# dropbox/rust-brotli

Hardware: AMD Instinct MI355X
Metric: compress MB/s at q5 lgwin22 (higher is better)
Workload: dtype u8; 1 GPU; 64 MiB synthetic English-like text per GPU, quality=5, lgwin=22, one-shot BrotliEncoderCompress (H6), input and stream resident in HBM; input_bytes_total=67108864, compressed_bytes=16370400

## Files before the change

### rust-brotli_amd/csrc/metablock_device.h

```cpp
#ifndef BROTLI_MI355X_METABLOCK_DEVICE_H_
#define BROTLI_MI355X_METABLOCK_DEVICE_H_

#include "lz77_chain.h"
#include "metablock_types.h"

namespace brotli_mi355x {

struct BitSink {
  uint64_t* words;
  uint64_t pos;
  BR_DEV void put(uint32_t n_bits, uint64_t bits) {
    if (n_bits == 0) return;
    const uint32_t sh = (uint32_t)(pos & 63u);
    uint64_t* w = words + (pos >> 6);
    w[0] |= bits << sh;
    if (sh + n_bits > 64) w[1] |= bits >> (64 - sh);
    pos += n_bits;
  }
};

#if defined(BR_CODES_PROFILE) && !defined(BROTLI_HOST_EMU)
static __device__ unsigned long long g_codes_prof[32];
struct CodesPhaseClock {
  unsigned long long last;
// ... 467 lines not shown
        total_reps_non_zero += reps;
        count_reps_non_zero++;
      }
      i += reps;
    }
    use_rle_for_non_zero = total_reps_non_zero > count_reps_non_zero * 2;
    use_rle_for_zero = total_reps_zero > count_reps_zero * 2;
  }
  uint32_t n = *tree_size;
  for (uint32_t i = 0; i < new_length;) {
    const uint8_t value = depth[i];
    uint32_t reps = 1;
    if ((value != 0 && use_rle_for_non_zero) || (value == 0 && use_rle_for_zero)) {
      for (uint32_t k = i + 1; k < new_length && depth[k] == value; ++k) reps++;
    }
    uint32_t repetitions = reps;
    if (value == 0) {
      if (repetitions == 11) {
        tree[n] = 0;
        extra[n] = 0;
        n++;
        repetitions--;
      }
      if (repetitions < 3) {
        for (uint32_t r = 0; r < repetitions; ++r) {
          tree[n] = 0;
          extra[n] = 0;
          n++;
        }
      } else {
        const uint32_t start = n;
        repetitions -= 3;
        for (;;) {
          tree[n] = 17;
          extra[n] = (uint8_t)(repetitions & 0x7);
          n++;
          repetitions >>= 3;
          if (repetitions == 0) break;
          repetitions--;
        }
        br_reverse_u8(tree, start, n);
        br_reverse_u8(extra, start, n);
      }
    } else {
      if (previous_value != value) {
        tree[n] = value;
        extra[n] = 0;
        n++;
        repetitions--;
      }
      if (repetitions == 7) {
        tree[n] = value;
        extra[n] = 0;
        n++;
        repetitions--;
      }
      if (repetitions < 3) {
        for (uint32_t r = 0; r < repetitions; ++r) {
          tree[n] = value;
          extra[n] = 0;
          n++;
        }
      } else {
        const uint32_t start = n;
        repetitions -= 3;
        for (;;) {
          tree[n] = 16;
          extra[n] = (uint8_t)(repetitions & 0x3);
          n++;
          repetitions >>= 2;
          if (repetitions == 0) break;
          repetitions--;
        }
        br_reverse_u8(tree, start, n);
        br_reverse_u8(extra, start, n);
      }
      previous_value = value;
    }
    i += reps;
  }
  *tree_size = n;
}

BR_DEV uint16_t br_reverse_bits(uint32_t num_bits, uint16_t bits) {
#if !defined(BROTLI_HOST_EMU)
  if (num_bits != 0) return (uint16_t)(__builtin_bitreverse32((uint32_t)bits) >> (32u - num_bits));
#endif
  const uint32_t kLut[16] = {0x0, 0x8, 0x4, 0xc, 0x2, 0xa, 0x6, 0xe, 0x1, 0x9, 0x5, 0xd, 0x3, 0xb, 0x7, 0xf};
  uint32_t retval = kLut[bits & 0xf];
  for (uint32_t i = 4; i < num_bits; i += 4) {
    retval <<= 4;
    bits = (uint16_t)(bits >> 4);
    retval |= kLut[bits & 0xf];
  }
  retval >>= ((0u - num_bits) & 0x3u);
  return (uint16_t)retval;
}
BR_DEV void br_convert_bit_depths_to_symbols(const uint8_t* depth, uint32_t len, uint16_t* bits) {
  uint16_t bl_count[16];
  uint16_t next_code[16];
  for (int i = 0; i < 16; ++i) bl_count[i] = 0;
  for (uint32_t i = 0; i < len; ++i) bl_count[depth[i]]++;
  bl_count[0] = 0;
  next_code[0] = 0;
  int code = 0;
  for (int i = 1; i < 16; ++i) {
    code = (code + bl_count[i - 1]) << 1;
    next_code[i] = (uint16_t)code;
  }
  for (uint32_t i = 0; i < len; ++i)
    if (depth[i] != 0) bits[i] = br_reverse_bits(depth[i], next_code[depth[i]]++);
}
#if !defined(BROTLI_HOST_EMU)
BR_DEV void br_convert_bit_depths_to_symbols_coop(const uint8_t* depth, uint32_t len, uint16_t* bits) {
  const uint32_t lane = threadIdx.x & 63u;
  const unsigned long long below = (1ull << lane) - 1ull;
  uint32_t cnt = 0;
  for (uint32_t base = 0; base < len; base += 64) {
    const uint32_t i = base + lane;
    const uint32_t d = i < len ? depth[i] : 0u;
#pragma unroll
    for (uint32_t k = 1; k < 16; ++k) {
      const unsigned long long m = __ballot(d == k);
      if (lane == k) cnt += (uint32_t)__popcll(m);
    }
  }
  uint32_t code = 0, running = 0;
#pragma unroll
  for (uint32_t k = 1; k < 16; ++k) {
    const uint32_t c_prev = k == 1 ? 0u : (uint32_t)__shfl((int)cnt, (int)(k - 1), 64);
    code = (code + c_prev) << 1;
    if (lane == k) running = code;
  }
  for (uint32_t base = 0; base < len; base += 64) {
    const uint32_t i = base + lane;
    const uint32_t d = i < len ? depth[i] : 0u;
    const uint32_t next = (uint32_t)__shfl((int)running, (int)d, 64);
    uint32_t rank = 0;
#pragma unroll
    for (uint32_t k = 1; k < 16; ++k) {
      const unsigned long long m = __ballot(d == k);
      if (d == k) rank = (uint32_t)__popcll(m & below);
      if (lane == k) running += (uint32_t)__popcll(m);
    }
    if (d != 0) bits[i] = br_reverse_bits(d, (uint16_t)(next + rank));
  }
  __threadfence_block();
  __builtin_amdgcn_wave_barrier();
}
#endif

struct HuffmanScratch {
  HuffmanTree tree[2 * 704 + 2];
  uint8_t rle_tree[704];
  uint8_t rle_extra[704];
  uint8_t good_for_rle[704];
  uint8_t pad[8];
  HuffmanTree sort_tmp[704];
};

BR_DEV void br_store_huffman_tree(const uint8_t* depths, uint32_t num, HuffmanScratch* sc, BitSink& out) {
  const uint8_t kStorageOrder[18] = {1, 2, 3, 4, 0, 5, 17, 6, 16, 7, 8, 9, 10, 11, 12, 13, 14, 15};
  const uint8_t kSymbols[6] = {0, 7, 3, 2, 1, 15};
  const uint8_t kBitLengths[6] = {2, 4, 3, 2, 2, 4};
  uint32_t huffman_tree_size = 0;
  uint8_t code_length_bitdepth[18];
  uint16_t code_length_bitdepth_symbols[18];
  uint32_t huffman_tree_histogram[18];
  for (int i = 0; i < 18; ++i) {
    code_length_bitdepth[i] = 0;
    code_length_bitdepth_symbols[i] = 0;
    huffman_tree_histogram[i] = 0;
  }
  BR_PHASE_CLOCK();
  br_write_huffman_tree(depths, num, &huffman_tree_size, sc->rle_tree, sc->rle_extra);
  BR_PHASE(4);
  for (uint32_t i = 0; i < huffman_tree_size; ++i) huffman_tree_histogram[sc->rle_tree[i]]++;
  BR_PHASE(5);
  int num_codes = 0;
  uint32_t code = 0;
  for (uint32_t i = 0; i < 18; ++i) {
    if (huffman_tree_histogram[i] != 0) {
      if (num_codes == 0) {
        code = i;
        num_codes = 1;
      } else if (num_codes == 1) {
        num_codes = 2;
        break;
      }
    }
  }
  br_create_huffman_tree(huffman_tree_histogram, 18, 5, sc->tree, code_length_bitdepth);
  br_convert_bit_depths_to_symbols(code_length_bitdepth, 18, code_length_bitdepth_symbols);
  {
    uint32_t skip_some = 0;
    uint32_t codes_to_store = 18;
    if (num_codes > 1) {
      for (; codes_to_store > 0; --codes_to_store)
        if (code_length_bitdepth[kStorageOrder[codes_to_store - 1]] != 0) break;
    }
    if (code_length_bitdepth[kStorageOrder[0]] == 0 && code_length_bitdepth[kStorageOrder[1]] == 0) {
      skip_some = 2;
      if (code_length_bitdepth[kStorageOrder[2]] == 0) skip_some = 3;
    }
    out.put(2, skip_some);
    for (uint32_t i = skip_some; i < codes_to_store; ++i) {
      const uint32_t l = code_length_bitdepth[kStorageOrder[i]];
      out.put(kBitLengths[l], kSymbols[l]);
    }
  }
  if (num_codes == 1) code_length_bitdepth[code] = 0;
  BR_PHASE(6);
  for (uint32_t i = 0; i < huffman_tree_size; ++i) {
    const uint32_t ix = sc->rle_tree[i];
    out.put(code_length_bitdepth[ix], code_length_bitdepth_symbols[ix]);
    if (ix == 16) {
      out.put(2, sc->rle_extra[i]);
    } else if (ix == 17) {
      out.put(3, sc->rle_extra[i]);
    }
  }
  BR_PHASE(7);
}

BR_DEV void br_build_and_store_huffman_tree(const uint32_t* histogram, uint32_t histogram_length, uint32_t alphabet_size,
                                            HuffmanScratch* sc, uint8_t* depth, uint16_t* bits, BitSink& out, bool coop = false) {
  uint32_t count = 0;
  uint32_t s4[4] = {0, 0, 0, 0};
  uint32_t max_bits = 0;
  for (uint32_t i = 0; i < histogram_length; ++i) {
    if (histogram[i] != 0) {
      if (count < 4) {
        s4[count] = i;
      } else if (count > 4) {
        break;
      }
      count++;
    }
  }
  for (uint32_t c = alphabet_size - 1; c != 0; c >>= 1) max_bits++;
  if (count <= 1) {
    out.put(4, 1);
    out.put(max_bits, s4[0]);
    depth[s4[0]] = 0;
    bits[s4[0]] = 0;
    return;
  }
  for (uint32_t i = 0; i < histogram_length; ++i) depth[i] = 0;
  BR_PHASE_CLOCK();
  br_create_huffman_tree(histogram, histogram_length, 15, sc->tree, depth, coop ? sc->sort_tmp : nullptr);
  BR_PHASE(14);
#if !defined(BROTLI_HOST_EMU)
  if (coop) br_convert_bit_depths_to_symbols_coop(depth, histogram_length, bits); else
#endif
  br_convert_bit_depths_to_symbols(depth, histogram_length, bits);
  BR_PHASE(8);
  if (count <= 4) {
    out.put(2, 1);
    out.put(2, count - 1);
    for (uint32_t i = 0; i < count; ++i) {
      for (uint32_t j = i + 1; j < count; ++j) {
        if (depth[s4[j]] < depth[s4[i]]) {
          const uint32_t t = s4[j];
          s4[j] = s4[i];
          s4[i] = t;
        }
      }
    }
    for (uint32_t i = 0; i < count; ++i) out.put(max_bits, s4[i]);
    if (count == 4) out.put(1, depth[s4[0]] == 1 ? 1 : 0);
  } else {
    br_store_huffman_tree(depth, histogram_length, sc, out);
  }
}

BR_DEV uint32_t br_block_length_offset(uint32_t code) {
  const uint32_t kOffset[26] = {1,   5,   9,   13,  17,  25,  33,  41,  49,   65,   81,   97,   113,
                                145, 177, 209, 241, 305, 369, 497, 753, 1265, 2289, 4337, 8433, 16625};
  return kOffset[code];
}
BR_DEV uint32_t br_block_length_nbits(uint32_t code) {
  const uint8_t kNbits[26] = {2, 2, 2, 2, 3, 3, 3, 3, 4, 4, 4, 4, 5, 5, 5, 5, 6, 6, 7, 8, 9, 10, 11, 12, 13, 24};
  return kNbits[code];
}
BR_DEV uint32_t br_block_length_prefix_code(uint32_t len) {
  uint32_t code = len >= 177 ? (len >= 753 ? 20 : 14) : (len >= 41 ? 7 : 0);
  while (code < 25 && len >= br_block_length_offset(code + 1)) code++;
  return code;
}
struct BlockTypeCodeCalculator {
  uint32_t last_type, second_last_type;
};
BR_DEV uint32_t br_next_block_type_code(BlockTypeCodeCalculator& c, uint8_t type) {
  const uint32_t type_code = (type == c.last_type + 1) ? 1u : (type == c.second_last_type ? 0u : (uint32_t)type + 2u);
  c.second_last_type = c.last_type;
  c.last_type = type;
  return type_code;
}
BR_DEV void br_store_var_len_uint8(uint32_t n, BitSink& out) {
  if (n == 0) {
    out.put(1, 0);
  } else {
    const uint32_t nbits = br_log2_floor_nonzero(n);
    out.put(1, 1);
    out.put(3, nbits);
    out.put(nbits, n - (1u << nbits));
  }
}

struct BlockSplitCode {
  uint8_t type_depths[258];
  uint16_t type_bits[258];
  uint8_t length_depths[26];
  uint16_t length_bits[26];
};

BR_DEV uint64_t br_block_switch_bits(const BlockSplitCode& code, uint32_t typecode, uint32_t block_len, bool is_first_block,
                                     uint32_t* nbits_out) {
  uint64_t bits = 0;
  uint32_t n = 0;
  if (!is_first_block) {
    bits = code.type_bits[typecode];
    n = code.type_depths[typecode];
  }
  const uint32_t lencode = br_block_length_prefix_code(block_len);
  bits |= (uint64_t)code.length_bits[lencode] << n;
  n += code.length_depths[lencode];
  bits |= (uint64_t)(block_len - br_block_length_offset(lencode)) << n;
  n += br_block_length_nbits(lencode);
  *nbits_out = n;
  return bits;
}

BR_DEV uint32_t br_block_type_code_at(const uint8_t* types, uint32_t i) {
  const uint32_t type = types[i];
  const uint32_t last = i >= 1 ? types[i - 1] : 1u;
  const uint32_t second_last = i >= 2 ? types[i - 2] : (i == 1 ? 1u : 0u);
  return (type == last + 1) ? 1u : (type == second_last ? 0u : type + 2u);
}
BR_DEV void br_build_and_store_block_split_code(const uint8_t* types, const uint32_t* lengths, uint32_t num_blocks,
                                                uint32_t num_types, HuffmanScratch* sc, BlockSplitCode* code,
                                                uint64_t* switch_bits, uint8_t* switch_nbits, BitSink& out,
                                                const uint32_t* histograms_in = nullptr) {
  uint32_t type_histo[258];
  uint32_t length_histo[26];
  BlockTypeCodeCalculator calc;
  if (histograms_in == nullptr) {
    for (int i = 0; i < 258; ++i) type_histo[i] = 0;
    for (int i = 0; i < 26; ++i) length_histo[i] = 0;
    calc.last_type = 1;
    calc.second_last_type = 0;
    for (uint32_t i = 0; i < num_blocks; ++i) {
      const uint32_t type_code = br_next_block_type_code(calc, types[i]);
      if (i != 0) type_histo[type_code]++;
      length_histo[br_block_length_prefix_code(lengths[i])]++;
// ... 224 lines not shown
```

### rust-brotli_amd/csrc/metablock_items.h

```cpp
#ifndef BROTLI_MI355X_METABLOCK_ITEMS_H_
#define BROTLI_MI355X_METABLOCK_ITEMS_H_

#include "metablock_fast.h"

#if defined(BROTLI_HOST_EMU)
#define BR_TID 0
#define BR_NT 1
#define BR_ATOMIC_ADD_U32(p, v) (*(p) += (v))
#define BR_ATOMIC_OR_U64(p, v) (*(p) |= (v))
#else
#define BR_TID ((int)threadIdx.x)
#define BR_NT ((int)blockDim.x)
#define BR_ATOMIC_ADD_U32(p, v) atomicAdd((p), (v))
#define BR_ATOMIC_OR_U64(p, v) atomicOr((unsigned long long*)(p), (unsigned long long)(v))
#endif

namespace brotli_mi355x {

struct MbBuffers {
  const uint8_t* text;
  const Command* cmds;
  uint32_t n_cmds, n_lits, n_dists, n_mb;
  uint32_t text_base;
  MbDesc* descs;
// ... 90 lines not shown
  }
  BR_SYNC();
  if (kind != kSplitDistance) {
    uint16_t* out = B.gran_hist[kind] + ((size_t)d.gran_row_base[kind] + (size_t)local_g * nc) * row;
    for (uint32_t j = BR_TID; j < nc * row; j += BR_NT) out[j] = (uint16_t)lds[j];
  }
}

BR_DEV void mb_item_distance_count(const MbBuffers& B, uint32_t c) {
  const Command cmd = B.cmds[c];
  if (!br_command_has_distance(cmd)) return;
  uint32_t lo = 0, hi = B.n_mb;
  while (hi - lo > 1) {
    const uint32_t mid = (lo + hi) >> 1;
    if (B.descs[mid].cmd_offset <= c) {
      lo = mid;
    } else {
      hi = mid;
    }
  }
  const MbDesc& d = B.descs[lo];
  if (d.uncompressed) return;
  const uint32_t local = B.cmd_dist_index[c] - d.dist_base;
  const uint32_t local_g = local / kDistanceGranule;
  uint16_t* rowp = B.gran_hist[kSplitDistance] + ((size_t)d.gran_row_base[kSplitDistance] + local_g) * kNumDistanceHistoSymbols;
  const uint32_t sym = cmd.dist_prefix_ & 0x3ffu;
  uint32_t* word = (uint32_t*)((uintptr_t)(rowp + sym) & ~(uintptr_t)3);
  const uint32_t shift = ((uintptr_t)(rowp + sym) & 2u) ? 16u : 0u;
  BR_ATOMIC_ADD_U32(word, 1u << shift);
}

static constexpr uint32_t kSplitRowMax = kMaxStaticContexts * 256 > 704 ? kMaxStaticContexts * 256 : 704;

struct SplitScratch {
  uint32_t curr[kSplitRowMax];
  uint32_t comb[2][kSplitRowMax];
  uint32_t last[2][kSplitRowMax];
  float terms[3][kSplitRowMax];
  float entropy[3 * kMaxStaticContexts];
  float last_entropy[2 * kMaxStaticContexts];
  uint32_t ctl[16];
};

BR_DEV void mb_rows_entropy(const EntropyTables& et, SplitScratch& S, uint32_t nc, uint32_t row, uint32_t alphabet) {
#if defined(BROTLI_HOST_EMU)
  const uint32_t lane = 0, lanes = 1, wave = 0, waves = 1;
#else
  const uint32_t lane = threadIdx.x & 63u, lanes = 64, wave = threadIdx.x >> 6, waves = blockDim.x >> 6;
#endif
  for (uint32_t r = wave; r < 3 * nc; r += waves) {
    const uint32_t w = r / nc, i = r % nc;
    const uint32_t* src = (w == 0 ? S.curr : S.comb[w - 1]) + i * row;
    float* out = S.terms[w] + i * row;
    uint32_t cnt = 0, total = 0;
    for (uint32_t base = 0; base < alphabet; base += lanes) {
      const uint32_t j = base + lane;
      const uint32_t p = j < alphabet ? src[j] : 0u;
      total += p;
      const bool nz = p != 0;
#if defined(BROTLI_HOST_EMU)
      if (nz) out[cnt] = (float)p * et.logs_16[p & 0xffffu];
      cnt += nz ? 1u : 0u;
#else
      const unsigned long long mask = __ballot(nz);
      const uint32_t before = (uint32_t)__popcll(mask & ((1ull << lane) - 1ull));
      if (nz) out[cnt + before] = (float)p * et.logs_16[p & 0xffffu];
      cnt += (uint32_t)__popcll(mask);
#endif
    }
#if !defined(BROTLI_HOST_EMU)
    for (int off = 32; off > 0; off >>= 1) total += __shfl_down(total, off, 64);
    __threadfence_block();
#endif
    if (lane == 0) {
      float retval = 0.0f;
      for (uint32_t n = 0; n < cnt; ++n) retval = retval - out[n];
      if (total != 0) retval = retval + (float)total * br_fast_log2(et, total);
      const float fsum = (float)total;
      S.entropy[r] = retval < fsum ? fsum : retval;
    }
  }
}

BR_DEV void mb_item_split_chain(const MbBuffers& B, uint32_t m, uint32_t kind, SplitScratch& S) {
  const MbDesc d = B.descs[m];
  if (d.uncompressed) return;
  const uint32_t row = kRowLen[kind];
  const uint32_t nc = kind == kSplitLiteral ? d.num_contexts : 1;
  const uint32_t entropy_alphabet = kind == kSplitDistance ? 64u : row;
  const uint32_t min_block = kGranuleLen[kind];
  const float threshold = kind == kSplitLiteral ? 400.0f : (kind == kSplitCommand ? 500.0f : 100.0f);
  const uint32_t max_types = kind == kSplitLiteral && nc > 1 ? 256u / nc : 256u;
  const uint32_t n_symbols = d.n_symbols[kind];
  const uint32_t n_gran = d.n_granules[kind];
  const uint16_t* G = B.gran_hist[kind] + (size_t)d.gran_row_base[kind] * row;
  uint32_t* H = B.histo[kind] + (size_t)d.histo_base[kind] * row;
  uint8_t* types = B.block_types[kind] + d.block_base[kind];
  uint32_t* lengths = B.block_lengths[kind] + d.block_base[kind];
  uint16_t* gran_block = B.gran_block[kind] + d.granule_base[kind];
  const uint32_t max_histos = d.max_histos[kind];
  const uint32_t W = nc * row;
  if (d.simple != 0) {
    for (uint32_t j = BR_TID; j < row; j += BR_NT) {
      uint32_t acc = 0;
      for (uint32_t q = 0; q < n_gran; ++q) acc += G[(size_t)q * row + j];
      H[j] = acc;
    }
    for (uint32_t q = BR_TID; q < n_gran; q += BR_NT) gran_block[q] = 0;
    if (BR_TID == 0) {
      types[0] = 0;
      lengths[0] = n_symbols;
      MbResult& r = B.results[m];
      r.num_types[kind] = 1;
      r.num_blocks[kind] = 1;
      r.num_histos[kind] = 1;
    }
    return;
  }

  uint32_t num_blocks = 0, num_types = 0, block_size = 0, target = min_block, curr_ix = 0, merge_count = 0;
  uint32_t last_ix[2] = {0, 0};
  uint32_t block_first_granule = 0;
  for (uint32_t j = BR_TID; j < W; j += BR_NT) {
    S.curr[j] = 0;
    S.last[0][j] = 0;
    S.last[1][j] = 0;
  }
  BR_SYNC();
  uint32_t g = 0;
  for (;;) {
    bool is_final = false;
    if (g < n_gran) {
      uint32_t m = (target - block_size) / min_block;
      if (m == 0) m = 1;
      if (m > n_gran - g) m = n_gran - g;
      const uint16_t* gr = G + (size_t)g * W;
      for (uint32_t j = BR_TID; j < W; j += BR_NT) {
        uint32_t acc = 0;
        uint32_t q = 0;
        for (; q + 4 <= m; q += 4) {
          const uint32_t a0 = gr[(size_t)q * W + j], a1 = gr[(size_t)(q + 1) * W + j], a2 = gr[(size_t)(q + 2) * W + j],
                         a3 = gr[(size_t)(q + 3) * W + j];
          acc += a0 + a1 + a2 + a3;
        }
        for (; q < m; ++q) acc += gr[(size_t)q * W + j];
        S.curr[j] += acc;
      }
      const uint64_t upto = (uint64_t)(g + m) * min_block;
      block_size += (uint32_t)((upto < n_symbols ? upto : n_symbols) - (uint64_t)g * min_block);
      g += m;
      BR_SYNC();
      if (block_size != target) continue;
    } else {
      is_final = true;
    }
    if (block_size < min_block) block_size = min_block;
    if (num_blocks == 0) {
      for (uint32_t i = BR_TID; i < nc; i += BR_NT) {
        const float e = br_bits_entropy(B.et, S.curr + i * row, entropy_alphabet);
        S.last_entropy[i] = e;
        S.last_entropy[nc + i] = e;
      }
      BR_SYNC();
      for (uint32_t j = BR_TID; j < W; j += BR_NT) {
        const uint32_t c = S.curr[j];
        H[j] = c;
        S.last[0][j] = c;
        S.last[1][j] = c;
        S.curr[j] = 0;
      }
      if (BR_TID == 0) {
        lengths[0] = block_size;
        types[0] = 0;
      }
      for (uint32_t q = block_first_granule + BR_TID; q < g; q += BR_NT) gran_block[q] = 0;
      block_first_granule = g;
      num_blocks = 1;
      num_types = 1;
      curr_ix += nc;
      block_size = 0;
      BR_SYNC();
    } else if (block_size > 0) {
      for (uint32_t j = BR_TID; j < W; j += BR_NT) {
        const uint32_t c = S.curr[j];
        S.comb[0][j] = c + S.last[0][j];
        S.comb[1][j] = c + S.last[1][j];
      }
      BR_SYNC();
      mb_rows_entropy(B.et, S, nc, row, entropy_alphabet);
      BR_SYNC();
      if (BR_TID == 0) {
        float diff[2] = {0.0f, 0.0f};
        for (uint32_t i = 0; i < nc; ++i) {
          for (uint32_t j = 0; j < 2; ++j) {
            const float v = S.entropy[(1 + j) * nc + i] - S.entropy[i] - S.last_entropy[j * nc + i];
            if (kind == kSplitLiteral && nc > 1) {
              diff[j] += v;
            } else {
              diff[j] = v;
            }
          }
        }
        uint32_t decision;
        if (num_types < max_types && diff[0] > threshold && diff[1] > threshold) {
          decision = 0;
        } else if (diff[1] < diff[0] - 20.0f) {
          decision = 1;
        } else {
          decision = 2;
        }
        S.ctl[0] = decision;
      }
      BR_SYNC();
      const uint32_t decision = S.ctl[0];
      BR_SYNC();
      if (decision == 0) {
        uint32_t* Hn = H + (size_t)curr_ix * row;
        const bool room = curr_ix + nc <= max_histos;
        for (uint32_t j = BR_TID; j < W; j += BR_NT) {
          const uint32_t c = S.curr[j];
          if (room) Hn[j] = c;
          S.last[1][j] = S.last[0][j];
          S.last[0][j] = c;
          S.curr[j] = 0;
        }
        if (BR_TID == 0) {
          lengths[num_blocks] = block_size;
          types[num_blocks] = (uint8_t)num_types;
          for (uint32_t i = 0; i < nc; ++i) {
            S.last_entropy[nc + i] = S.last_entropy[i];
            S.last_entropy[i] = S.entropy[i];
          }
        }
        for (uint32_t q = block_first_granule + BR_TID; q < g; q += BR_NT) gran_block[q] = (uint16_t)num_blocks;
        last_ix[1] = last_ix[0];
        last_ix[0] = (kind == kSplitLiteral && nc > 1) ? num_types * nc : (num_types & 0xffu);
        num_blocks++;
        num_types++;
        curr_ix += nc;
        block_size = 0;
        merge_count = 0;
        target = min_block;
      } else if (decision == 1) {
        const uint32_t t = last_ix[0];
        last_ix[0] = last_ix[1];
        last_ix[1] = t;
        uint32_t* Hl = H + (size_t)last_ix[0] * row;
        for (uint32_t j = BR_TID; j < W; j += BR_NT) {
          const uint32_t merged = S.comb[1][j];
          Hl[j] = merged;
          S.last[1][j] = S.last[0][j];
          S.last[0][j] = merged;
          S.curr[j] = 0;
        }
        if (BR_TID == 0) {
          lengths[num_blocks] = block_size;
          types[num_blocks] = types[num_blocks - 2];
          for (uint32_t i = 0; i < nc; ++i) {
            S.last_entropy[nc + i] = S.last_entropy[i];
            S.last_entropy[i] = S.entropy[2 * nc + i];
          }
        }
        for (uint32_t q = block_first_granule + BR_TID; q < g; q += BR_NT) gran_block[q] = (uint16_t)num_blocks;
        num_blocks++;
        block_size = 0;
        merge_count = 0;
        target = min_block;
      } else {
        uint32_t* Hl = H + (size_t)last_ix[0] * row;
        const bool single_type = num_types == 1;
        for (uint32_t j = BR_TID; j < W; j += BR_NT) {
          const uint32_t merged = S.comb[0][j];
          Hl[j] = merged;
          S.last[0][j] = merged;
          if (single_type) S.last[1][j] = merged;
          S.curr[j] = 0;
        }
        if (BR_TID == 0) {
          lengths[num_blocks - 1] += block_size;
          for (uint32_t i = 0; i < nc; ++i) {
            S.last_entropy[i] = S.entropy[nc + i];
            if (num_types == 1) S.last_entropy[nc + i] = S.last_entropy[i];
          }
        }
        for (uint32_t q = block_first_granule + BR_TID; q < g; q += BR_NT) gran_block[q] = (uint16_t)(num_blocks - 1);
        block_size = 0;
        if (++merge_count > 1) target += min_block;
      }
      block_first_granule = g;
      BR_SYNC();
    }
    if (is_final) break;
  }
  if (BR_TID == 0) {
    MbResult& r = B.results[m];
    r.num_types[kind] = num_types;
    r.num_blocks[kind] = num_blocks;
    r.num_histos[kind] = num_types * nc;
  }
}

BR_DEV uint32_t mb_build_code_core(uint32_t kind, uint32_t num_distance_symbols, uint32_t* h, uint8_t* depth, uint16_t* bits,
                                   uint64_t* words, HuffmanScratch* sc, bool coop = false, uint32_t mode = kCodeOptimized) {
  const uint32_t row = kRowLen[kind];
  if (mode == kCodeFast || mode == kCodeStatic) {
    for (uint32_t i = 0; i < row; ++i) {
      depth[i] = 0;
      bits[i] = 0;
    }
    for (uint32_t i = 0; i < kTreeBitsWords; ++i) words[i] = 0;
    BitSink sink;
    sink.words = words;
    sink.pos = 0;
    if (mode == kCodeStatic) {
      br_store_static_code(kind, depth, bits, sink);
    } else {
      uint32_t total = 0;
      for (uint32_t i = 0; i < row; ++i) total += h[i];
      const uint32_t max_bits = kind == kSplitLiteral ? 8u : (kind == kSplitCommand ? 10u : br_log2_floor_nonzero(num_distance_symbols - 1u) + 1u);
      br_build_and_store_huffman_tree_fast(h, total, max_bits, sc, depth, bits, sink);
    }
    return (uint32_t)sink.pos;
  }
  uint32_t opt_len = row;
  if (kind == kSplitDistance) opt_len = num_distance_symbols < kNumDistanceHistoSymbols ? num_distance_symbols : kNumDistanceHistoSymbols;
  BR_PHASE_CLOCK();
  if (mode == kCodeOptimized) br_optimize_huffman_counts_for_rle(opt_len, h, sc->good_for_rle, coop);
  BR_PHASE(9);
  uint32_t hist_len = row, alphabet = row;
  if (kind == kSplitDistance) {
    hist_len = num_distance_symbols < kNumDistanceHistoSymbols ? num_distance_symbols : kNumDistanceHistoSymbols;
    alphabet = num_distance_symbols;
  }
  for (uint32_t i = 0; i < row; ++i) {
    depth[i] = 0;
    bits[i] = 0;
  }
  for (uint32_t i = 0; i < kTreeBitsWords; ++i) words[i] = 0;
  BitSink sink;
  sink.words = words;
  sink.pos = 0;
  BR_PHASE(10);
  br_build_and_store_huffman_tree(h, hist_len, alphabet, sc, depth, bits, sink, coop);
  BR_PHASE(11);
  return (uint32_t)sink.pos;
}

BR_DEV void mb_item_build_code(const MbBuffers& B, uint32_t kind, uint32_t row_index, uint32_t num_distance_symbols,
                               HuffmanScratch* sc, uint32_t mode = kCodeOptimized) {
  const uint32_t row = kRowLen[kind];
  B.tree_nbits[kind][row_index] =
      mb_build_code_core(kind, num_distance_symbols, B.histo[kind] + (size_t)row_index * row, B.depth[kind] + (size_t)row_index * row,
                         B.bits[kind] + (size_t)row_index * row, B.tree_bits[kind] + (size_t)row_index * kTreeBitsWords, sc, false, mode);
}

BR_DEV void mb_append_bits(BitSink& out, const uint64_t* words, uint32_t nbits) {
  uint32_t i = 0;
  while (nbits >= 32) {
    out.put(32, (words[i >> 1] >> ((i & 1) * 32)) & 0xffffffffull);
    nbits -= 32;
    i++;
  }
  if (nbits) out.put(nbits, (words[i >> 1] >> ((i & 1) * 32)) & ((1ull << nbits) - 1));
}

struct MbSplitPrepared {
  uint32_t histograms[3][258 + 26];
  BlockSplitCode code[3];
};
BR_DEV void mb_item_write_header(const MbBuffers& B, uint32_t m, HuffmanScratch* sc, uint64_t* staging = nullptr, MbSplitPrepared* prepared = nullptr) {
  const MbDesc d = B.descs[m];
  MbResult& r = B.results[m];
  if (d.uncompressed) {
    r.header_bits = 0;
    return;
  }
// ... 309 lines not shown
```

### rust-brotli_amd/csrc/metablock_kernels.hip

```cpp
#include <hip/hip_runtime.h>

#include "device_api.h"
#include "device_scan.h"
#include "metablock_api.h"
#include "metablock_hq.h"

namespace brotli_mi355x {

size_t mb_scan_scratch_bytes(size_t n) { return scan_scratch_words(n) * 4 + 256; }

template <typename F>
__global__ __launch_bounds__(256) void k_for_each(uint32_t n, F f) {
  const uint32_t i = blockIdx.x * blockDim.x + threadIdx.x;
  if (i < n) f(i);
}
template <typename F>
static void for_each(uint32_t n, F f) {
  if (n == 0) return;
  hipLaunchKernelGGL(k_for_each<F>, dim3((n + 255) / 256), dim3(256), 0, BR_STREAM, n, f);
}

void mb_gather_at_metablock_starts(const MbBuffers& B, const uint32_t* src, uint32_t* out_dev) {
  const MbBuffers b = B;
  for_each(b.n_mb + 1, [b, src, out_dev] __device__(uint32_t m) { out_dev[m] = src[m < b.n_mb ? b.descs[m].cmd_offset : b.n_cmds]; });
// ... 32 lines not shown
  const uint32_t m = blockIdx.y;
  const MbDesc d = B.descs[m];
  const uint32_t length = d.end - d.start;
  const uint32_t n_strides = length >= 64 ? (length - 64) / 4096 + 1 : 0;
  const uint32_t wave = threadIdx.x >> 6, lane = threadIdx.x & 63, n_waves = kStatsChunks * 4;
  if (blockIdx.x * 4 >= n_strides) return;
  for (uint32_t j = threadIdx.x; j < kContextStatsWords; j += blockDim.x) s[j] = 0;
  __syncthreads();
  const uint8_t* text = B.text + d.start + lane;
  constexpr uint32_t kBatch = 4;
  for (uint32_t t0 = blockIdx.x * 4 + wave; t0 < n_strides; t0 += n_waves * kBatch) {
    uint32_t bytes[kBatch];
    for (uint32_t u = 0; u < kBatch; ++u) {
      const uint32_t t = t0 + u * n_waves;
      bytes[u] = t < n_strides ? text[(size_t)t * 4096] : 0u;
    }
    for (uint32_t u = 0; u < kBatch; ++u) {
      if (t0 + u * n_waves >= n_strides) break;
      const uint32_t literal = bytes[u];
      const uint32_t prev1 = (uint32_t)__shfl_up((int)literal, 1, 64), prev2 = (uint32_t)__shfl_up((int)literal, 2, 64);
      {
        const uint32_t lut = 0x90u;
        const uint32_t bin = ((lut >> ((prev1 >> 6) * 2)) & 3u) * 3u + ((lut >> ((literal >> 6) * 2)) & 3u);
        uint32_t mine = 0;
        for (uint32_t b = 0; b < 9; ++b) {
          const uint32_t count = (uint32_t)__popcll(__ballot(lane >= 1 && bin == b));
          if (lane == b) mine = count;
        }
        if (mine) atomicAdd(&s[lane], mine);
      }
      if (lane >= 2) {
        const uint32_t context = br_static_context_map(3, br_context(B.utf8_lut, B.signed_lut, (uint8_t)prev1, (uint8_t)prev2, 2));
        atomicAdd(&s[48 + context * 32 + (literal >> 3)], 1u);
      }
      if (lane == 0) atomicAdd(&s[480], 62u);
    }
  }
  __syncthreads();
  uint32_t* row = stats + (size_t)m * kContextStatsWords;
  for (uint32_t j = threadIdx.x; j < kContextStatsWords; j += blockDim.x) {
    uint32_t v = s[j];
    if (j >= 16 && j < 48)
      for (uint32_t c = 0; c < 13; ++c) v += s[48 + c * 32 + (j - 16)];
    if (v) atomicAdd(&row[j], v);
  }
}

void mb_context_stats(const MbBuffers& B, uint32_t* stats_dev) {
  if (B.n_mb == 0) return;
  for (uint32_t first = 0; first < B.n_mb; first += 32768) {
    MbBuffers b = B;
    b.descs += first;
    const uint32_t n = B.n_mb - first < 32768 ? B.n_mb - first : 32768;
    hipLaunchKernelGGL(k_context_stats, dim3(kStatsChunks, n), dim3(256), 0, BR_STREAM, b, stats_dev + (size_t)first * kContextStatsWords);
  }
  HIP_CHECK(hipGetLastError());
}

__global__ __launch_bounds__(256) void k_granule_histograms(MbBuffers B, uint32_t kind) {
  __shared__ uint32_t lds[kMaxStaticContexts * 256];
  mb_item_granule_histogram(B, kind, blockIdx.x, lds);
}

void mb_granule_histograms(const MbBuffers& B) {
  const MbBuffers b = B;
  if (b.n_granules[kSplitLiteral]) hipLaunchKernelGGL(k_granule_histograms, dim3(b.n_granules[kSplitLiteral]), dim3(256), 0, BR_STREAM, b, (uint32_t)kSplitLiteral);
  if (b.n_granules[kSplitCommand]) hipLaunchKernelGGL(k_granule_histograms, dim3(b.n_granules[kSplitCommand]), dim3(256), 0, BR_STREAM, b, (uint32_t)kSplitCommand);
  if (b.n_granules[kSplitDistance]) {
    dev_memset(b.gran_hist[kSplitDistance], 0, (size_t)b.n_granules[kSplitDistance] * kNumDistanceHistoSymbols * 2);
    for_each(b.n_cmds, [b] __device__(uint32_t c) { mb_item_distance_count(b, c); });
  }
  HIP_CHECK(hipGetLastError());
}

__global__ __launch_bounds__(1024) void k_split_chains(MbBuffers B) {
  __shared__ SplitScratch S;
  mb_item_split_chain(B, blockIdx.x / 3, blockIdx.x % 3, S);
}

void mb_split_chains(const MbBuffers& B, bool wide) {
  if (B.n_mb == 0) return;
  hipLaunchKernelGGL(k_split_chains, dim3(B.n_mb * 3), dim3(wide ? 1024 : 256), 0, BR_STREAM, B);
  HIP_CHECK(hipGetLastError());
}

__global__ __launch_bounds__(64) void k_build_codes(MbBuffers B, const CodeJob* jobs, uint32_t n_jobs) {
  __shared__ HuffmanScratch sc;
  __shared__ uint32_t h[704];
  __shared__ uint16_t bits[704];
  __shared__ uint8_t depth[704];
  __shared__ uint64_t words[kTreeBitsWords];
  __shared__ uint32_t nbits;
  const uint32_t i = blockIdx.x;
  if (i >= n_jobs) return;
  const CodeJob j = jobs[i];
  const uint32_t row = kRowLen[j.kind];
  uint32_t* gh = B.histo[j.kind] + (size_t)j.row_index * row;
  for (uint32_t k = threadIdx.x; k < row; k += 64) h[k] = gh[k];
  __syncthreads();
  {
    const uint32_t nb = mb_build_code_core(j.kind, j.num_distance_symbols, h, depth, bits, words, &sc, true, j.mode);
    if (threadIdx.x == 0) nbits = nb;
  }
  __syncthreads();
  uint8_t* gd = B.depth[j.kind] + (size_t)j.row_index * row;
  uint16_t* gb = B.bits[j.kind] + (size_t)j.row_index * row;
  uint64_t* gw = B.tree_bits[j.kind] + (size_t)j.row_index * kTreeBitsWords;
  for (uint32_t k = threadIdx.x; k < row; k += 64) {
    gh[k] = h[k];
    gd[k] = depth[k];
    gb[k] = bits[k];
  }
  for (uint32_t k = threadIdx.x; k < kTreeBitsWords; k += 64) gw[k] = words[k];
  if (threadIdx.x == 0) B.tree_nbits[j.kind][j.row_index] = nbits;
}

void mb_build_codes(const MbBuffers& B, const CodeJob* jobs_dev, uint32_t n_jobs) {
  if (n_jobs == 0) return;
  hipLaunchKernelGGL(k_build_codes, dim3(n_jobs), dim3(64), 0, BR_STREAM, B, jobs_dev, n_jobs);
  HIP_CHECK(hipGetLastError());
#if defined(BR_CODES_PROFILE)
  {
    unsigned long long h[32];
    HIP_CHECK(hipStreamSynchronize(BR_STREAM));
    HIP_CHECK(hipMemcpyFromSymbol(h, HIP_SYMBOL(g_codes_prof), sizeof(h)));
    fprintf(stderr, "codes profile (%u jobs), cycles sum / slowest job:", n_jobs);
    for (int i = 0; i < 16; ++i) fprintf(stderr, " [%d] %llu / %llu", i, h[i], h[16 + i]);
    fprintf(stderr, "\n");
    unsigned long long z[32] = {0};
    HIP_CHECK(hipMemcpyToSymbol(HIP_SYMBOL(g_codes_prof), z, sizeof(z)));
  }
#endif
}

__global__ __launch_bounds__(64) void k_write_headers(MbBuffers B) {
  constexpr uint32_t kLdsWords = 5120;
  constexpr uint64_t kOtherBits = 160u * 1024u;
  __shared__ uint64_t lw[kLdsWords];
  __shared__ HuffmanScratch sc_lds;
  __shared__ MbSplitPrepared prep;
  __shared__ uint32_t s_bits;
  const uint32_t m = blockIdx.x;
  if (m >= B.n_mb) return;
  const MbDesc d = B.descs[m];
  uint64_t* global_words = B.header_words + (size_t)m * B.header_stride;
  if (d.uncompressed) {
    if (threadIdx.x == 0) mb_item_write_header(B, m, B.huff_scratch + m, global_words);
    return;
  }
  uint32_t trees = 0;
  for (uint32_t kind = 0; kind < 3; ++kind)
    for (uint32_t i = threadIdx.x; i < B.results[m].num_histos[kind]; i += 64) trees += B.tree_nbits[kind][d.histo_base[kind] + i];
  for (int off = 32; off > 0; off >>= 1) trees += __shfl_down(trees, off, 64);
  trees = (uint32_t)__shfl((int)trees, 0, 64);
  const bool in_lds = (uint64_t)trees + kOtherBits <= (uint64_t)kLdsWords * 64;
  uint64_t* stage = in_lds ? lw : global_words;
  const uint32_t clear_words = in_lds ? kLdsWords : B.header_stride;
  for (uint32_t i = threadIdx.x; i < clear_words; i += 64) stage[i] = 0;
  for (uint32_t i = threadIdx.x; i < 3 * (258 + 26); i += 64) (&prep.histograms[0][0])[i] = 0;
  __syncthreads();
  for (uint32_t kind = 0; kind < 3; ++kind) {
    const uint8_t* types = B.block_types[kind] + d.block_base[kind];
    const uint32_t* lengths = B.block_lengths[kind] + d.block_base[kind];
    const uint32_t nb = B.results[m].num_blocks[kind];
    for (uint32_t i = threadIdx.x; i < nb; i += 64) {
      if (i != 0) atomicAdd(&prep.histograms[kind][br_block_type_code_at(types, i)], 1u);
// ... 270 lines not shown
```

Before: 4491 MB/s.

## Parallelize Huffman tree RLE writing and storage across a wavefront

Adds a wave-cooperative path for writing the RLE-coded Huffman tree, building its code-length histogram, and emitting its bits. It uses ballots and prefix scans over 64 lanes, and places bits with atomicOr at prefix-summed positions. This replaces serial per-symbol loops in k_build_codes when coop is set, which k_build_codes passes as true. It also adds optional split-chain profiling that is compiled out by default. Risks include wavefront-only assumptions, a fixed 11-chunk limit, and possible bit-exactness bugs in the RLE logic.

```diff
diff --git a/rust-brotli_amd/csrc/metablock_device.h b/rust-brotli_amd/csrc/metablock_device.h
--- a/rust-brotli_amd/csrc/metablock_device.h
+++ b/rust-brotli_amd/csrc/metablock_device.h
@@ -573,6 +573,181 @@
   *tree_size = n;
 }
 
+#if !defined(BROTLI_HOST_EMU) && !defined(BR_NO_COOP_TREE_WRITER)
+
+BR_DEV uint32_t br_tree_run_entries(uint32_t value, uint32_t reps, uint32_t prev, uint8_t* tree, uint8_t* extra) {
+  const bool zero = value == 0;
+  uint32_t literals = 0;
+  if (zero ? reps == 11 : prev != value) {
+    literals++;
+    reps--;
+  }
+  if (!zero && reps == 7) {
+    literals++;
+    reps--;
+  }
+  const bool coded = reps >= 3;
+  if (!coded) literals += reps;
+  if (tree != nullptr) {
+    for (uint32_t k = 0; k < literals; ++k) {
+      tree[k] = (uint8_t)value;
+      extra[k] = 0;
+    }
+  }
+  if (!coded) return literals;
+  const uint32_t shift = zero ? 3u : 2u;
+  uint32_t rest = reps - 3, digits = 1;
+  for (uint32_t t = rest >> shift; t != 0; t = (t - 1) >> shift) digits++;
+  if (tree != nullptr) {
+    for (uint32_t k = digits; k-- != 0;) {
+      tree[literals + k] = zero ? 17 : 16;
+      extra[literals + k] = (uint8_t)(rest & ((1u << shift) - 1u));
+      rest = (rest >> shift) - 1u;
+    }
+  }
+  return literals + digits;
+}
+
+BR_DEV uint32_t br_wave_scan_max(uint32_t x, uint32_t lane) {
+#pragma unroll
+  for (int off = 1; off < 64; off <<= 1) {
+    const uint32_t y = (uint32_t)__shfl_up((int)x, off, 64);
+    if ((int)lane >= off) x = x > y ? x : y;
+  }
+  return x;
+}
+BR_DEV uint32_t br_wave_scan_add(uint32_t x, uint32_t lane) {
+#pragma unroll
+  for (int off = 1; off < 64; off <<= 1) {
+    const uint32_t y = (uint32_t)__shfl_up((int)x, off, 64);
+    if ((int)lane >= off) x += y;
+  }
+  return x;
+}
+BR_DEV uint32_t br_wave_sum(uint32_t x) {
+#pragma unroll
+  for (int off = 32; off > 0; off >>= 1) x += (uint32_t)__shfl_xor((int)x, off, 64);
+  return x;
+}
+
+BR_DEV void br_write_huffman_tree_coop(const uint8_t* depth, uint32_t length, uint32_t* tree_size, uint8_t* tree, uint8_t* extra) {
+  const uint32_t lane = threadIdx.x & 63u;
+  length = (uint32_t)__builtin_amdgcn_readfirstlane((int)length);
+  uint32_t new_length = 0;
+  for (uint32_t base = 0; base < length; base += 64) {
+    const uint32_t i = base + lane;
+    const unsigned long long m = __ballot(i < length && depth[i] != 0);
+    if (m != 0) new_length = base + 64u - (uint32_t)__builtin_clzll(m);
+  }
+  new_length = (uint32_t)__builtin_amdgcn_readfirstlane((int)new_length);
+  const uint32_t chunks = (new_length + 63u) / 64u;
+  uint32_t rs[11];
+  uint32_t total_reps_zero = 0, total_reps_non_zero = 0, count_reps_zero = 0, count_reps_non_zero = 0;
+  {
+    uint32_t carry = 0;
+#pragma unroll
+    for (uint32_t c = 0; c < 11; ++c) {
+      rs[c] = 0;
+      if (c >= chunks) continue;
+      const uint32_t i = c * 64u + lane;
+      const bool in = i < new_length;
+      const uint32_t d = in ? depth[i] : 0u;
+      const bool starts = in && (i == 0 || depth[i - 1] != d);
+      uint32_t x = br_wave_scan_max(starts ? i : 0u, lane);
+      x = x > carry ? x : carry;
+      rs[c] = x;
+      carry = (uint32_t)__shfl((int)x, 63, 64);
+      const bool ends = in && (i + 1 == new_length || depth[i + 1] != d);
+      const uint32_t reps = i - x + 1u;
+      if (ends && reps >= 3 && d == 0) {
+        total_reps_zero += reps;
+        count_reps_zero++;
+      }
+      if (ends && reps >= 4 && d != 0) {
+        total_reps_non_zero += reps;
+        count_reps_non_zero++;
+      }
+    }
+  }
+  bool use_rle_for_non_zero = false, use_rle_for_zero = false;
+  if (length > 50) {
+    use_rle_for_non_zero = br_wave_sum(total_reps_non_zero) > (br_wave_sum(count_reps_non_zero) + 1u) * 2u;
+    use_rle_for_zero = br_wave_sum(total_reps_zero) > (br_wave_sum(count_reps_zero) + 1u) * 2u;
+  }
+  uint32_t n = *tree_size;
+  uint32_t prev_carry = 0;
+#pragma unroll
+  for (uint32_t c = 0; c < 11; ++c) {
+    if (c >= chunks) continue;
+    const uint32_t i = c * 64u + lane;
+    const bool in = i < new_length;
+    const uint32_t d = in ? depth[i] : 0u;
+    const bool rle = d != 0 ? use_rle_for_non_zero : use_rle_for_zero;
+    const bool ends = in && (i + 1 == new_length || depth[i + 1] != d);
+    const bool owner = in && (!rle || ends);
+    const uint32_t reps = rle ? i - rs[c] + 1u : 1u;
+    const uint32_t key = br_wave_scan_max((owner && d != 0) ? (((i + 1u) << 8) | d) : 0u, lane);
+    uint32_t before = (uint32_t)__shfl_up((int)key, 1, 64);
+    if (lane == 0) before = 0;
+    before = before > prev_carry ? before : prev_carry;
+    const uint32_t last = (uint32_t)__shfl((int)key, 63, 64);
+    prev_carry = last > prev_carry ? last : prev_carry;
+    const uint32_t prev = before != 0 ? (before & 0xffu) : 8u;
+    const uint32_t count = owner ? br_tree_run_entries(d, reps, prev, nullptr, nullptr) : 0u;
+    const uint32_t upto = br_wave_scan_add(count, lane);
+    if (owner) br_tree_run_entries(d, reps, prev, tree + n + upto - count, extra + n + upto - count);
+    n += (uint32_t)__shfl((int)upto, 63, 64);
+  }
+  *tree_size = n;
+  __threadfence_block();
+  __builtin_amdgcn_wave_barrier();
+}
+
+BR_DEV void br_tree_histogram_coop(const uint8_t* tree, uint32_t n, uint32_t* histogram) {
+  const uint32_t lane = threadIdx.x & 63u;
+  for (uint32_t base = 0; base < n; base += 64) {
+    const uint32_t i = base + lane;
+    const uint32_t s = i < n ? tree[i] : 0xffu;
+#pragma unroll
+    for (uint32_t k = 0; k < 18; ++k) histogram[k] += (uint32_t)__popcll(__ballot(s == k));
+  }
+}
+
+BR_DEV void br_store_tree_entries_coop(const uint8_t* tree, const uint8_t* extra, uint32_t n, const uint8_t* code_depth,
+                                       const uint16_t* code_symbols, BitSink& out) {
+  const uint32_t lane = threadIdx.x & 63u;
+  uint32_t mine = 0;
+#pragma unroll
+  for (uint32_t k = 0; k < 18; ++k)
+    if (lane == k) mine = (uint32_t)code_depth[k] | ((uint32_t)code_symbols[k] << 8);
+  __threadfence_block();
+  __builtin_amdgcn_wave_barrier();
+  uint64_t pos = out.pos;
+  for (uint32_t base = 0; base < n; base += 64) {
+    const uint32_t i = base + lane;
+    const bool in = i < n;
+    const uint32_t ix = in ? tree[i] : 0u;
+    const uint32_t code = (uint32_t)__shfl((int)mine, (int)ix, 64);
+    const uint32_t code_bits = code & 0xffu;
+    const uint32_t extra_bits = ix == 16 ? 2u : (ix == 17 ? 3u : 0u);
+    const uint32_t width = in ? code_bits + extra_bits : 0u;
+    const uint32_t upto = br_wave_scan_add(width, lane);
+    if (width != 0) {
+      const uint64_t bits = (uint64_t)((code >> 8) | (extra_bits != 0 ? (uint32_t)extra[i] << code_bits : 0u));
+      const uint64_t at = pos + upto - width;
+      const uint32_t sh = (uint32_t)(at & 63u);
+      unsigned long long* w = (unsigned long long*)out.words + (at >> 6);
+      atomicOr(w, (unsigned long long)(bits << sh));
+      if (sh + width > 64) atomicOr(w + 1, (unsigned long long)(bits >> (64 - sh)));
+    }
+    pos += (uint32_t)__shfl((int)upto, 63, 64);
+  }
+  out.pos = pos;
+  __threadfence_block();
+  __builtin_amdgcn_wave_barrier();
+}
+#endif
+
 BR_DEV uint16_t br_reverse_bits(uint32_t num_bits, uint16_t bits) {
 #if !defined(BROTLI_HOST_EMU)
   if (num_bits != 0) return (uint16_t)(__builtin_bitreverse32((uint32_t)bits) >> (32u - num_bits));
@@ -650,7 +825,7 @@
   HuffmanTree sort_tmp[704];
 };
 
-BR_DEV void br_store_huffman_tree(const uint8_t* depths, uint32_t num, HuffmanScratch* sc, BitSink& out) {
+BR_DEV void br_store_huffman_tree(const uint8_t* depths, uint32_t num, HuffmanScratch* sc, BitSink& out, bool coop = false) {
   const uint8_t kStorageOrder[18] = {1, 2, 3, 4, 0, 5, 17, 6, 16, 7, 8, 9, 10, 11, 12, 13, 14, 15};
   const uint8_t kSymbols[6] = {0, 7, 3, 2, 1, 15};
   const uint8_t kBitLengths[6] = {2, 4, 3, 2, 2, 4};
@@ -664,9 +839,18 @@
     huffman_tree_histogram[i] = 0;
   }
   BR_PHASE_CLOCK();
-  br_write_huffman_tree(depths, num, &huffman_tree_size, sc->rle_tree, sc->rle_extra);
-  BR_PHASE(4);
-  for (uint32_t i = 0; i < huffman_tree_size; ++i) huffman_tree_histogram[sc->rle_tree[i]]++;
+#if !defined(BROTLI_HOST_EMU) && !defined(BR_NO_COOP_TREE_WRITER)
+  if (coop) {
+    br_write_huffman_tree_coop(depths, num, &huffman_tree_size, sc->rle_tree, sc->rle_extra);
+    BR_PHASE(4);
+    br_tree_histogram_coop(sc->rle_tree, huffman_tree_size, huffman_tree_histogram);
+  } else
+#endif
+  {
+    br_write_huffman_tree(depths, num, &huffman_tree_size, sc->rle_tree, sc->rle_extra);
+    BR_PHASE(4);
+    for (uint32_t i = 0; i < huffman_tree_size; ++i) huffman_tree_histogram[sc->rle_tree[i]]++;
+  }
   BR_PHASE(5);
   int num_codes = 0;
   uint32_t code = 0;
@@ -702,6 +886,13 @@
   }
   if (num_codes == 1) code_length_bitdepth[code] = 0;
   BR_PHASE(6);
+#if !defined(BROTLI_HOST_EMU) && !defined(BR_NO_COOP_TREE_WRITER)
+  if (coop) {
+    br_store_tree_entries_coop(sc->rle_tree, sc->rle_extra, huffman_tree_size, code_length_bitdepth, code_length_bitdepth_symbols, out);
+    BR_PHASE(7);
+    return;
+  }
+#endif
   for (uint32_t i = 0; i < huffman_tree_size; ++i) {
     const uint32_t ix = sc->rle_tree[i];
     out.put(code_length_bitdepth[ix], code_length_bitdepth_symbols[ix]);
@@ -761,7 +952,7 @@
     for (uint32_t i = 0; i < count; ++i) out.put(max_bits, s4[i]);
     if (count == 4) out.put(1, depth[s4[0]] == 1 ? 1 : 0);
   } else {
-    br_store_huffman_tree(depth, histogram_length, sc, out);
+    br_store_huffman_tree(depth, histogram_length, sc, out, coop);
   }
 }
 
diff --git a/rust-brotli_amd/csrc/metablock_items.h b/rust-brotli_amd/csrc/metablock_items.h
--- a/rust-brotli_amd/csrc/metablock_items.h
+++ b/rust-brotli_amd/csrc/metablock_items.h
@@ -196,6 +196,38 @@
   }
 }
 
+#if defined(BR_SPLIT_PROFILE) && !defined(BROTLI_HOST_EMU)
+static constexpr uint32_t kSplitProfChains = 64;
+static __device__ unsigned long long g_split_prof[3][4];
+static __device__ unsigned long long g_split_prof_chain[kSplitProfChains][3][4];
+struct SplitPhaseClock {
+  unsigned long long last, cycles[3], decisions;
+  BR_DEV SplitPhaseClock() : last(__builtin_readcyclecounter()), cycles{0, 0, 0}, decisions(0) {}
+  BR_DEV void mark(int phase) {
+    const unsigned long long now = __builtin_readcyclecounter();
+    cycles[phase] += now - last;
+    last = now;
+  }
+  BR_DEV void flush(uint32_t m, uint32_t kind) {
+    if (threadIdx.x != 0) return;
+    for (int p = 0; p < 4; ++p) {
+      const unsigned long long v = p < 3 ? cycles[p] : decisions;
+      atomicAdd(&g_split_prof[kind][p], v);
+      if (m < kSplitProfChains) g_split_prof_chain[m][kind][p] = v;
+    }
+  }
+};
+#define BR_SPLIT_CLOCK() SplitPhaseClock br_split_clock
+#define BR_SPLIT_PHASE(k) br_split_clock.mark(k)
+#define BR_SPLIT_DECISION() br_split_clock.decisions++
+#define BR_SPLIT_FLUSH(m, kind) br_split_clock.flush(m, kind)
+#else
+#define BR_SPLIT_CLOCK()
+#define BR_SPLIT_PHASE(k)
+#define BR_SPLIT_DECISION()
+#define BR_SPLIT_FLUSH(m, kind)
+#endif
+
 BR_DEV void mb_item_split_chain(const MbBuffers& B, uint32_t m, uint32_t kind, SplitScratch& S) {
   const MbDesc d = B.descs[m];
   if (d.uncompressed) return;
@@ -241,9 +273,11 @@
     S.last[1][j] = 0;
   }
   BR_SYNC();
+  BR_SPLIT_CLOCK();
   uint32_t g = 0;
   for (;;) {
     bool is_final = false;
+    BR_SPLIT_PHASE(2);
     if (g < n_gran) {
       uint32_t m = (target - block_size) / min_block;
       if (m == 0) m = 1;
@@ -264,6 +298,7 @@
       block_size += (uint32_t)((upto < n_symbols ? upto : n_symbols) - (uint64_t)g * min_block);
       g += m;
       BR_SYNC();
+      BR_SPLIT_PHASE(0);
       if (block_size != target) continue;
     } else {
       is_final = true;
@@ -276,6 +311,7 @@
         S.last_entropy[nc + i] = e;
       }
       BR_SYNC();
+      BR_SPLIT_PHASE(1);
       for (uint32_t j = BR_TID; j < W; j += BR_NT) {
         const uint32_t c = S.curr[j];
         H[j] = c;
@@ -328,6 +364,8 @@
       BR_SYNC();
       const uint32_t decision = S.ctl[0];
       BR_SYNC();
+      BR_SPLIT_PHASE(1);
+      BR_SPLIT_DECISION();
       if (decision == 0) {
         uint32_t* Hn = H + (size_t)curr_ix * row;
         const bool room = curr_ix + nc <= max_histos;
@@ -406,6 +444,8 @@
     }
     if (is_final) break;
   }
+  BR_SPLIT_PHASE(2);
+  BR_SPLIT_FLUSH(m, kind);
   if (BR_TID == 0) {
     MbResult& r = B.results[m];
     r.num_types[kind] = num_types;
diff --git a/rust-brotli_amd/csrc/metablock_kernels.hip b/rust-brotli_amd/csrc/metablock_kernels.hip
--- a/rust-brotli_amd/csrc/metablock_kernels.hip
+++ b/rust-brotli_amd/csrc/metablock_kernels.hip
@@ -138,6 +138,35 @@
   if (B.n_mb == 0) return;
   hipLaunchKernelGGL(k_split_chains, dim3(B.n_mb * 3), dim3(wide ? 1024 : 256), 0, BR_STREAM, B);
   HIP_CHECK(hipGetLastError());
+#if defined(BR_SPLIT_PROFILE)
+  {
+    static unsigned long long sums[3][4], chains[kSplitProfChains][3][4];
+    HIP_CHECK(hipStreamSynchronize(BR_STREAM));
+    HIP_CHECK(hipMemcpyFromSymbol(sums, HIP_SYMBOL(g_split_prof), sizeof(sums)));
+    HIP_CHECK(hipMemcpyFromSymbol(chains, HIP_SYMBOL(g_split_prof_chain), sizeof(chains)));
+    const uint32_t n = B.n_mb < kSplitProfChains ? B.n_mb : kSplitProfChains;
+    for (uint32_t kind = 0; kind < 3; ++kind) {
+      uint32_t slowest = 0;
+      unsigned long long most = 0;
+      for (uint32_t m = 0; m < n; ++m) {
+        const unsigned long long t = chains[m][kind][0] + chains[m][kind][1] + chains[m][kind][2];
+        if (t > most) {
+          most = t;
+          slowest = m;
+        }
+      }
+      const unsigned long long* c = chains[slowest][kind];
+      fprintf(stderr, "split profile (%u meta-blocks, %u threads) kind %u, cycles: all chains sums %llu entropy+decision %llu commit %llu (%llu decisions); "
+              "slowest chain m=%u sums %llu entropy+decision %llu commit %llu (%llu decisions), sums are %.1f %% of it\n",
+              B.n_mb, wide ? 1024u : 256u, kind, sums[kind][0], sums[kind][1], sums[kind][2], sums[kind][3], slowest, c[0], c[1], c[2], c[3],
+              most ? 100.0 * (double)c[0] / (double)most : 0.0);
+    }
+    for (size_t i = 0; i < sizeof(sums) / sizeof(unsigned long long); ++i) (&sums[0][0])[i] = 0;
+    for (size_t i = 0; i < sizeof(chains) / sizeof(unsigned long long); ++i) (&chains[0][0][0])[i] = 0;
+    HIP_CHECK(hipMemcpyToSymbol(HIP_SYMBOL(g_split_prof), sums, sizeof(sums)));
+    HIP_CHECK(hipMemcpyToSymbol(HIP_SYMBOL(g_split_prof_chain), chains, sizeof(chains)));
+  }
+#endif
 }
 
 __global__ __launch_bounds__(64) void k_build_codes(MbBuffers B, const CodeJob* jobs, uint32_t n_jobs) {
```

After: 4494 MB/s (median of 4 runs). About the same (+0.1%).
